# JGCRI/xanthos

Measured on AMD Instinct MI355X. Metric: cell-months/sec (pm_abcd_mrtm, 67,420 cells), higher is better.
Workload: dtype f64

## Files before the change

### xanthos_amd/csrc/xh_flow_rsum.cpp

```cpp
#include <algorithm>
#include <cstdio>
#include <numeric>
#include <string>
#include <thread>

#include "xh_flow_plan.h"

using xh_flow::Tree;
using xh_flow::tree_analyse;

namespace {

constexpr int LANES = 64;
constexpr int G_MAX = 16;
constexpr int W_MAX = 9;
constexpr int SK_P = 4;
constexpr unsigned SK_ZERO = 2u * LANES * 16u;
constexpr int H_MAX = 88;

struct RPart {
    std::vector<int> queue, piece, roots, psize, pimp, pdepth;
    std::vector<int> e_prod, e_cons, e_kind;
    std::vector<int> unit_of_piece, unit_cells, unit_imp, unit_out, unit_depth;
    std::vector<char> unit_cheap, unit_special, special, mayfire;
    int nunit = 0, nedge = 0, maxdepth = 0, n_cheap = 0;
    int n_special = -1;
};

void rsum_partition(const Tree &t, const FlowPlanOptions &opt, int cap, RPart &P, std::vector<int> &fold_leaf) {
    const int n = t.n;
    const std::vector<int> &ds = t.ds, &child = t.child, &child_ptr = t.child_ptr;
    P = RPart();
    std::vector<int> &queue = P.queue;
    queue.reserve(n);
// ... 279 lines not shown
    for (int pass = 0; pass < 4 && need > 0 && opt.foldable; ++pass) {
        std::vector<int> gain(npiece, 0);
        for (int c : queue) {
            const int q = P.piece[c];
            if (q < 0 || special[c] || fold_leaf[c] >= 0 || P.pimp[q] != 0) continue;
            for (int k = child_ptr[c]; k < child_ptr[c + 1]; ++k)
                if (opt.foldable[child[k]] && t.nchild[child[k]] == 0 && P.piece[child[k]] == q) {
                    gain[q]++;
                    break;
                }
        }
        std::vector<int> order;
        for (int p = 0; p < npiece; ++p)
            if (gain[p] > 0) order.push_back(p);
        std::stable_sort(order.begin(), order.end(), [&](int x, int y) { return gain[x] > gain[y]; });
        const int want = (need + 1) * LANES + LANES / 2;
        std::vector<char> chosen(npiece, 0);
        int got = 0;
        for (int p : order) {
            if (got >= want) break;
            chosen[p] = 1;
            got += gain[p];
        }
        if (got == 0) break;
        fold_pieces([&](int p) { return chosen[p] != 0; });
        mark_folds();
        need = pack(false);
    }
    if (need > 0) pack(true);
}

}

int flow_rsum_planner_version() { return 8; }

int flow_tables_build_rsum(int n, const int64_t *indptr, const int32_t *indices, const int8_t *sign, const int *comp,
                           int ncomp, const FlowPlanOptions &opt, std::vector<char> &handled, FlowTables &out,
                           std::string &err) {
    out = FlowTables();
    out.rsum = true;
    handled.assign(n, 0);
    if (n == 0) return 0;
    Tree t;
    tree_analyse(n, indptr, indices, sign, comp, ncomp, t);
    const std::vector<int> &ds = t.ds;

    RPart P;
    std::vector<int> fold_leaf;
    {
        static const int caps[] = {LANES, 56, 48, 44, 40, 36, 32, 28, 24};
        constexpr int NCAP = (int)(sizeof(caps) / sizeof(caps[0]));
        std::vector<RPart> cand(opt.piece_cap > 0 ? 1 : NCAP);
        std::vector<std::vector<int>> cand_fold(cand.size());
        if (cand.size() == 1 || n < 4096) {
            for (size_t k = 0; k < cand.size(); ++k)
                rsum_partition(t, opt, opt.piece_cap > 0 ? std::min(opt.piece_cap, LANES) : caps[k], cand[k], cand_fold[k]);
        } else {
            std::vector<std::thread> pool;
            for (size_t k = 0; k < cand.size(); ++k) pool.emplace_back([&, k] { rsum_partition(t, opt, caps[k], cand[k], cand_fold[k]); });
            for (auto &th : pool) th.join();
        }
        bool have = false;
        long best_score = 0;
        for (size_t k = 0; k < cand.size(); ++k) {
            RPart &Q = cand[k];
            int indep = 0;
            for (int u = 0; u < Q.nunit; ++u) indep += (Q.unit_imp[u] == 0 && Q.unit_out[u] == 0) ? 1 : 0;
// ... 185 lines not shown
    out.n_edges = nedge;
    out.depth = P.maxdepth + 1;
    out.n_cells = (int)std::count(handled.begin(), handled.end(), (char)1);
    out.max_imports = *std::max_element(P.unit_imp.begin(), P.unit_imp.end());
    out.max_exports = *std::max_element(unit_exp.begin(), unit_exp.end());
    out.edge_prod_cell = P.e_prod;
    out.edge_cons_cell = P.e_cons;
    out.unit_depth = P.unit_depth;
    out.piece_of_cell = piece;
    out.unit_of_cell.assign(n, -1);
    for (int c = 0; c < n; ++c)
        if (piece[c] >= 0) out.unit_of_cell[c] = unit_of_piece[piece[c]];
    out.height_of_cell = hgt;
    out.ds = ds;

    if (opt.debug) {
        std::vector<int> hs(4, 0), hl(14, 0), hi(6, 0);
        int indep = 0;
        for (int u = 0; u < nunit; ++u) {
            hs[out.unit_p[u] & 3]++;
            hl[std::min(out.unit_lmax[u] / 16, 13)]++;
            hi[P.unit_imp[u] == 0 ? 0 : P.unit_imp[u] <= 2 ? 1 : P.unit_imp[u] <= 4 ? 2 : P.unit_imp[u] <= 8 ? 3 : 4]++;
            indep += (P.unit_imp[u] == 0 && unit_exp[u] == 0) ? 1 : 0;
        }
        fprintf(stderr, "flow plan (reassociated): %d units (%d without streams, %d kept cheap), %d pieces, %d streams, depth %d, %lld of %lld lanes used\n",
                nunit, indep, P.n_cheap, (int)roots.size(), nedge, P.maxdepth + 1, (long long)out.n_cells, (long long)ts);
        {
            int nfu = 0, nfi = 0;
            for (int u = 0; u < nunit; ++u) {
                nfu += (out.unit_p[u] & 4) ? 1 : 0;
                nfi += ((out.unit_p[u] & 4) && (P.unit_imp[u] > 0 || unit_exp[u] > 0)) ? 1 : 0;
            }
            fprintf(stderr, "  folded leaves: %d, in %d units (of them with streams: %d)\n", out.n_folded, nfu, nfi);
        }
        {
            int nsu = 0;
            for (int u = 0; u < nunit; ++u) nsu += (out.unit_p[u] & 16) ? 1 : 0;
            int nx = 0;
            for (int c = 0; c < n; ++c) nx += (P.n_special >= 0 && P.mayfire[c]) ? 1 : 0;
            int quiet = 0;
            for (int u = 0; u < nunit && P.n_special >= 0; ++u) {
                bool any = (out.unit_p[u] & 16) != 0;
                for (int k = 0; k < LANES && !any; ++k) any = (out.lane_flags[(int64_t)u * LANES + k] & 1) != 0;
                quiet += any ? 0 : 1;
            }
            for (int u = 0; u < nunit && P.n_special >= 0; ++u)
                if (out.unit_p[u] & 16)
                    fprintf(stderr, "  pair unit %d: %d cells, %d imports, %d outlets, depth %d, lmax %d\n", u, P.unit_cells[u], P.unit_imp[u], unit_exp[u],
                            P.unit_depth[u], out.unit_lmax[u]);
            fprintf(stderr, "  single-sum plan: %s, %d cells may fire, %d of them in pair form in %d units; %d single units hold no cell that may fire\n",
                    P.n_special >= 0 ? "yes" : "no", nx, std::max(P.n_special, 0), nsu, quiet);
        }
        fprintf(stderr, "  units by reads (none, A, R, A+R): %d %d %d %d\n  units by lmax/16 (0..13+):", hs[0], hs[1], hs[2], hs[3]);
        for (int k = 0; k < 14; ++k) fprintf(stderr, " %d", hl[k]);
        fprintf(stderr, "\n  units by imports (0, <=2, <=4, <=8, more): %d %d %d %d %d\n  longest stream jump: %d levels\n", hi[0], hi[1],
                hi[2], hi[3], hi[4], out.skew_span);
    }
    return 0;
}

std::string flow_tables_check_rsum(int n, const int64_t *indptr, const int32_t *indices, const int8_t *sign,
                                   const std::vector<char> &handled, const FlowTables &t) {
    if (!t.rsum) return "not a reassociated plan";
    if (t.n_units == 0) {
        for (int c = 0; c < n; ++c)
            if (handled[c]) return "handled cell without units";
// ... 167 lines not shown
```

### xanthos_amd/csrc/xh_mrtm.hip

```cpp
#include <algorithm>
#include <chrono>
#include <climits>
#include <cmath>
#include <atomic>
#include <numeric>
#include <thread>

#include "xh_common.h"
#include <sys/stat.h>
#include <unistd.h>

#include "xh_mrtm_flow.h"
#include "xh_mrtm_plan.h"

namespace {

constexpr int W_MAX = 9;
constexpr int W_BASE = 3;
constexpr int UNIT_MAX_CELLS = 3072;
constexpr int BIN_CELLS = 256;
constexpr int N_CLASS = XH_ROUTE_N_CLASS;

struct UnitClass {
    int nt, kc;
// ... 677 lines not shown
    info[2] = plan->n_units;
    info[3] = plan->fb.n;
    info[4] = plan->largest_unit;
    info[5] = plan->total_slots;
    info[6] = plan->fb_all.single_ds ? 1 : 0;
    const FlowPlan *exact = plan->form[XH_FORM_EXACT].fp, *rsum = last_reassoc(plan);
    int64_t fi[5];
    flow_plan_info(rsum ? rsum : exact, fi);
    info[7] = fi[0];
    info[8] = fi[1];
    info[9] = fi[2];
    info[10] = fi[3];
    info[11] = fi[4];
    info[12] = rsum ? rsum->skew_lmax : ((exact && exact->skew_ok) ? exact->skew_lmax : -1);
    info[13] = plan->last.kernel;
    info[14] = plan->reroutes;
    info[15] = plan->validated;
    return XH_OK;
}

extern "C" int xh_route_plan_stats(xh_route_plan *plan, int64_t max_words, uint64_t *h_words, int64_t *n_words) {
    if (!plan || !n_words) return XH_ERR_ARG;
    std::vector<unsigned long long> st;
    const FlowPlan *rsum = last_reassoc(plan);
    int rc = flow_stats_fetch(plan->ctx, const_cast<FlowPlan *>(rsum ? rsum : plan->form[XH_FORM_EXACT].fp), st);
    if (rc) return rc;
    *n_words = (int64_t)st.size();
    if (h_words)
        for (int64_t i = 0; i < (int64_t)st.size() && i < max_words; ++i) h_words[i] = st[i];
    return XH_OK;
}

constexpr double CAPABLE_THRESHOLD = 1.0 - 1.0 / 1048576.0;

void xh_route_confirm(const xh_route_record &r) { r.plan->fault_streak = 0; }

extern "C" int xh_route_plan_prepare(xh_ctx *ctx, xh_route_plan *plan, const double *h_flow_dist, const double *h_velocity,
                                     double dt) {
    if (!ctx || !plan) return XH_ERR_ARG;
    XH_REQUIRE(ctx, plan->ctx == ctx, "xh_route_plan_prepare: plan belongs to another context");
    XH_REQUIRE(ctx, h_flow_dist && h_velocity && dt > 0.0, "xh_route_plan_prepare: bad argument");
    XH_HIP(ctx, hipSetDevice(ctx->device));
    if (reassoc_wanted(0)) {
        static const bool fold_on = xh_env_on("XH_FLOW_FOLD", true), single_on = xh_env_on("XH_RSUM_SINGLE", true);
        if ((!fold_on && !single_on) || !plan->form[XH_FORM_EXACT].fp || plan->h_indptr.empty()) return XH_OK;
        const size_t n = (size_t)plan->ncell;
        std::vector<unsigned char> foldable(n, 0), capable(n, 0);
        size_t nfold = 0;
        uint64_t key = XH_FNV_BASIS;
        for (size_t c = 0; c < n; ++c) {
            const double tauinv = h_velocity[c] / h_flow_dist[c];
            const bool leaf = plan->h_indptr[c + 1] - plan->h_indptr[c] == 1;
            capable[c] = (tauinv * dt <= CAPABLE_THRESHOLD) ? 0 : 1;
            foldable[c] = (leaf && tauinv >= 0.0 && tauinv * dt <= CAPABLE_THRESHOLD) ? 1 : 0;
            nfold += foldable[c];
            const unsigned char sets = (unsigned char)(capable[c] | (foldable[c] << 1));
            key = xh_fnv1a(key, &sets, 1);
        }
        key = xh_fnv1a(key, &dt, sizeof(dt));
        if (key == 0) key = 1;
        if (plan->fold_tried && key == plan->prep_key) return XH_OK;
        RouteForm &prepared = plan->form[XH_FORM_PREPARED];
        if (prepared.fp) {
            XH_HIP(ctx, hipStreamSynchronize(ctx->stream));
            if (plan->last.fp == prepared.fp) {
                plan->last.form = XH_FORM_EXACT;
                plan->last.fp = nullptr;
            }
            flow_plan_destroy(prepared.fp);
            prepared.fp = nullptr;
            prepared.first_checked = false;
        }
        plan->fold_tried = true;
        plan->prep_key = key;
        plan->fold_disabled = false;
        const bool fold = fold_on && nfold > 0;
        if (!fold && !single_on) return XH_OK;
        const int rcu = rsum_partition(ctx, plan, fold ? foldable.data() : nullptr, single_on ? capable.data() : nullptr,
                                       &prepared.fp);
        if (rcu || !prepared.fp) return rcu;
        prepared.suffix = prepared.fp->n_special >= 0 ? "_rs" : "_rf";
        plan->fold_dt = dt;
        return XH_OK;
    }
    return XH_OK;
}

// ... 254 lines not shown
```

### xanthos_amd/csrc/xh_mrtm_flow.hip

```cpp

#include <algorithm>
#include <cmath>
#include <cstdlib>
#include <numeric>

#include "xh_flow_plan.h"
#include "xh_mrtm_flow.h"

namespace {

constexpr int W_MAX = 9;
constexpr int LANES = 64;
constexpr int NPAIR = 2 * LANES + 1;
constexpr int RING = 4;
constexpr int PF = 8;
constexpr unsigned FAULT_DATA_WAIT = 1, FAULT_RING_WAIT = 2;
constexpr unsigned FAULT_TEST = 99;
constexpr unsigned long long SPIN_LIMIT_TICKS = 500000000ull;

struct FlowArgs {
    const int *cell_of_slot;
    const unsigned *ent;
    const int *export_edge;
    const int *ghost_edge;
// ... 217 lines not shown
int put(xh_ctx *ctx, FlowBuf &b, const std::vector<T> &v) {
    XH_HIP(ctx, hipMalloc(&b.p, v.empty() ? 16 : v.size() * sizeof(T)));
    if (!v.empty()) XH_HIP(ctx, hipMemcpy(b.p, v.data(), v.size() * sizeof(T), hipMemcpyHostToDevice));
    return XH_OK;
}

}

void flow_plan_destroy(FlowPlan *fp) {
    if (!fp) return;
    FlowBuf *bufs[] = {&fp->d_cell_of_slot, &fp->d_ent,      &fp->d_export_edge, &fp->d_ghost_edge,
                       &fp->d_edge_cons_unit, &fp->d_unit_terms, &fp->d_lag,        &fp->d_ghost_lag,
                       &fp->d_ent2,         &fp->d_eprev,       &fp->d_unit_order,  &fp->d_unit_p,     &fp->d_unit_lmax,   &fp->d_unit_glmax,
                       &fp->d_lane_flags,   &fp->d_fold_cell};
    for (FlowBuf *b : bufs)
        if (b->p) (void)hipFree(b->p);
    if (fp->d_x) (void)hipFree(fp->d_x);
    if (fp->d_skew_args) (void)hipFree(fp->d_skew_args);
    if (fp->d_stats) (void)hipFree(fp->d_stats);
    delete fp;
}

void flow_plan_info(const FlowPlan *fp, int64_t info[5]) {
    info[0] = fp ? fp->n_units : 0;
    info[1] = fp ? fp->n_edges : 0;
    info[2] = fp ? fp->depth : 0;
    info[3] = fp ? fp->n_cells : 0;
    info[4] = fp ? fp->max_imports : 0;
}

FlowPlanOptions flow_plan_options(const xh_ctx *ctx) {
    FlowPlanOptions o;
    o.simds = 4 * (ctx->prop.multiProcessorCount > 0 ? ctx->prop.multiProcessorCount : 0);
    if (const char *e = getenv("XH_FLOW_PIECE_CAP")) o.piece_cap = std::min(std::max(atoi(e), 1), LANES);
    o.debug = xh_flow_debug();
    return o;
}

int flow_tables_host(FlowPlanOptions opt, int n, const int64_t *indptr, const int32_t *indices, const int8_t *sign,
                     const std::vector<int> &comp, int ncomp, std::vector<char> &handled, FlowTables &t, std::string &err) {
    handled.assign(n, 0);
    t = FlowTables();
    if (n == 0) return 0;
    opt.capable = nullptr;
    if (flow_tables_build(n, indptr, indices, sign, comp.data(), ncomp, opt, handled, t, err) != 0) return -1;
    if (t.n_units == 0) return 0;
    if (xh_flow_check()) {
        const std::string bad = flow_tables_check(n, indptr, indices, sign, handled, t);
        if (!bad.empty()) {
            err = "flow plan check: " + bad;
            return -1;
        }
    }
    return 0;
}

int flow_tables_cached(const char *name, int n, const int64_t *indptr, const int32_t *indices, const int8_t *sign, bool rsum,
                       bool folds, bool singles, FlowTables &t, std::vector<char> &handled,
                       const std::function<int(FlowTables &, std::vector<char> &)> &build) {
    const std::string path = name ? xh_cache_path(name, false) : std::string();
    if (!path.empty() && flow_tables_load(path.c_str(), t) && t.rsum == rsum && t.n_units > 0 &&
        (int64_t)t.cell_of_slot.size() == (int64_t)t.n_units * LANES && (folds || t.n_folded == 0) && (singles || t.n_special < 0)) {
        handled.assign((size_t)n, 0);
        bool ok = true;
        for (const std::vector<int> *cells : {&t.cell_of_slot, &t.fold_of_slot})
            for (int c : *cells) {
// ... 160 lines not shown
```

### xanthos_amd/csrc/xh_mrtm_rsum.hip

```cpp
#include <algorithm>
#include "xh_mrtm_wave_unit.h"

namespace {

__global__ void __launch_bounds__(LANES) __attribute__((amdgpu_waves_per_eu(2, 2))) k_mrtm_rsum(const WaveArgs *ap_) {
    WaveArgsK *ap = (WaveArgsK *)ap_;
    __shared__ __attribute__((aligned(16))) v2d lds[RING * NSLOT];
    __shared__ uint2 xtab[LANES];
    __shared__ unsigned qstage_sh[4 * LANES];
    __shared__ double fend_sh[2 * LANES];
    __shared__ int unit_sh, prio_sh;
    const int unit = wave_claim(ap, &unit_sh, &prio_sh);
    const int prio = prio_sh;
    if (unit < 0) return;
    if (A(months_ready)) {
        if (prio == 3) __builtin_amdgcn_s_setprio(3);
        else if (prio == 1) __builtin_amdgcn_s_setprio(1);
        else __builtin_amdgcn_s_setprio(2);
    } else if (prio == 3) {
        __builtin_amdgcn_s_setprio(3);
    }
    const int p = A(unit_p)[unit];
    const bool has_ghost = A(ghost_edge)[(int64_t)unit * LANES + threadIdx.x] >= 0;
    const bool g = __any(has_ghost), g2 = __any(has_ghost && threadIdx.x >= 8);
    const int nxo = __popcll(__ballot(A(export_edge)[(int64_t)unit * LANES + threadIdx.x] >= 0));
    const bool x = nxo > 0;
    char *l = reinterpret_cast<char *>(lds);
    __attribute__((address_space(3))) unsigned *qst = (__attribute__((address_space(3))) unsigned *)qstage_sh;
    __attribute__((address_space(3))) double *fnd = (__attribute__((address_space(3))) double *)fend_sh;
    fend_sh[threadIdx.x] = 0.0;
    fend_sh[LANES + threadIdx.x] = 0.0;
    if ((p & ~31) != 0x400) {
        if (threadIdx.x == 0) __hip_atomic_store(A(fault), FAULT_PLACE_WAIT, __ATOMIC_RELAXED, __HIP_MEMORY_SCOPE_AGENT);
        return;
    }
    bool bad = false;
#define XH_BY_OUTLETS(...)                                                                 \
    do {                                                                                   \
        if (nxo > 8) wave_unit<__VA_ARGS__, -1>(ap, l, xtab, qst, fnd, unit);              \
        else if (x) wave_unit<__VA_ARGS__, 1>(ap, l, xtab, qst, fnd, unit);                \
        else wave_unit<__VA_ARGS__, 0>(ap, l, xtab, qst, fnd, unit);                       \
    } while (0)
    if (p & 16) {
        if (!(p & 8) || (p & 4)) bad = true;
        else if (g2) XH_BY_OUTLETS(1, 0, 2, true, true, false, 2);
        else if (g) XH_BY_OUTLETS(1, 0, 1, true, true, false, 2);
        else XH_BY_OUTLETS(1, 0, 0, true, true, false, 2);
#undef XH_BY_OUTLETS
    } else if (p & 8) {
        if (p & 4) {
            if (g || !A(fold_cell)) bad = true;
            else wave_unit<1, 0, 0, true, true, true, 1>(ap, l, xtab, qst, fnd, unit);
        } else if (g2) wave_unit<1, 0, 2, true, true, false, 1>(ap, l, xtab, qst, fnd, unit);
        else if (g) wave_unit<1, 0, 1, true, true, false, 1>(ap, l, xtab, qst, fnd, unit);
        else if ((p & 2) || x) wave_unit<1, 0, 0, true, true, false, 1>(ap, l, xtab, qst, fnd, unit);
        else if (p & 1) wave_unit<1, 0, 0, false, true, false, 1>(ap, l, xtab, qst, fnd, unit);
        else wave_unit<0, 0, 0, false, true, false, 1>(ap, l, xtab, qst, fnd, unit);
    } else if (p & 4) {
        if (g || !A(fold_cell)) bad = true;
        else wave_unit<1, 0, 0, true, true, true>(ap, l, xtab, qst, fnd, unit);
    } else if (g2) wave_unit<1, 0, 2, true, true>(ap, l, xtab, qst, fnd, unit);
    else if (g) wave_unit<1, 0, 1, true, true>(ap, l, xtab, qst, fnd, unit);
    else if ((p & 2) || x) wave_unit<1, 0, 0, true, true>(ap, l, xtab, qst, fnd, unit);
    else if (p & 1) wave_unit<1, 0, 0, false, true>(ap, l, xtab, qst, fnd, unit);
    else wave_unit<0, 0, 0, false, true>(ap, l, xtab, qst, fnd, unit);
    if (bad && threadIdx.x == 0)
        __hip_atomic_store(A(fault), FAULT_PLACE_WAIT, __ATOMIC_RELAXED, __HIP_MEMORY_SCOPE_AGENT);
}
#undef A

}

const void *wave_rsum_kernel() { return reinterpret_cast<const void *>(&k_mrtm_rsum); }
```

### xanthos_amd/csrc/xh_mrtm_wave_unit.h

```cpp
#pragma once
#include <algorithm>
#include <climits>
#include <cstdlib>
#include <type_traits>

#include "xh_mrtm_flow.h"

namespace {


constexpr int LANES = 64;
constexpr int SK_P = 4;
#ifndef XH_WAVE_MIDZONE
#define XH_WAVE_MIDZONE 1
#endif
#ifndef XH_WAVE_BMOV
#define XH_WAVE_BMOV 1
#endif
constexpr int NSLOT = 2 * LANES + 1;
constexpr int RING = 8;
constexpr int GROUP = 16;
constexpr int SK_R = 2;
#ifndef XH_WAVE_CH
#define XH_WAVE_CH 256
// ... 116 lines not shown
template <int PRE, int POST, int NG, bool CHAIN, bool RSUM = false, bool FOLD = false, int SGL = 0, int NXR = -1>
__device__ __forceinline__ void wave_unit(WaveArgsK *ap, char *lds_generic, uint2 *xtab,
                                          __attribute__((address_space(3))) unsigned *qstage,
                                          __attribute__((address_space(3))) double *fend, const int unit) {
    constexpr bool HAS_G = NG > 0;
    constexpr bool V8 = SGL == 1;
    typedef Val<V8> V;
    typedef typename V::T val_t;
    typedef typename V::lds_c lds_cv;
    typedef typename V::lds_m lds_mv;
    constexpr unsigned VB = V::B;
    constexpr unsigned SLOTB = NSLOT * VB;
    lds_char *lds0 = (lds_char *)lds_generic;
    const int lane = threadIdx.x;
    const int64_t slot = (int64_t)unit * LANES + lane;

    const int gc = A(cell_of_slot)[slot];
    const bool valid = gc >= 0;
    const int gc_safe = valid ? gc : 0;
    const unsigned row_off = (unsigned)gc_safe * A(q_row_stride);
    const double tauinv = valid ? A(velocity)[gc] / A(flow_dist)[gc] : 0.0;
    const double acoef = 1.0 - tauinv * A(dt);
    const double area = valid ? A(area)[gc] : 0.0;
    const double S0v = (valid && A(S0)) ? A(S0)[gc] : 0.0;
    auto ent_off = [](unsigned o) { return V8 ? o >> 1 : o; };
    static_assert(!RSUM || (PRE <= 1 && POST == 0), "reassociated form: one inflow entry");
    static_assert(!FOLD || (RSUM && NG == 0), "folded leaves: reassociated form, units without imports");
    static_assert(SGL == 0 || RSUM, "single-sum plans: reassociated form");
    const int gcL = FOLD ? A(fold_cell)[slot] : -1;
    const bool validL = FOLD && valid && gcL >= 0;
    const unsigned row_offL = (unsigned)(validL ? gcL : 0) * A(q_row_stride);
    const double tauL = validL ? A(velocity)[gcL] / A(flow_dist)[gcL] : 0.0;
    const double acoefL = 1.0 - tauL * A(dt);
    const double areaL = validL ? A(area)[gcL] : 0.0;
    const double S0L = (validL && A(S0)) ? A(S0)[gcL] : 0.0;
    double SL = 0.0, favgL = 0.0, erlL = 0.0, erlL_n = 0.0, snapSL = 0.0, snapAL = 0.0, FL = 0.0;
    constexpr double FOLD_EPS = 1e-6;
    unsigned gfold = (validL && !(tauL * A(dt) <= 1.0 - 1.0 / 1048576.0 && tauL >= 0.0 && S0L >= 0.0)) ? 1u : 0u;
    constexpr double SGL_EPS = 1e-6;
    constexpr double SGL_XEPS = 1e-10;
    unsigned gsgl = 0;
    bool xlane = false;
    double fmin_seen = 0.0;
    if (SGL != 0) {
        const unsigned lf = A(lane_flags)[slot];
        xlane = valid && (lf & 2u) != 0;
        gsgl = (valid && (!(tauinv >= 0.0) || (!(tauinv * A(dt) <= 1.0 - 1.0 / 1048576.0) && !(lf & 1u)) || S0v < 0.0)) ? 1u : 0u;
    }
    constexpr int PRE_N = PRE > 0 ? PRE : 1, POST_N = POST > 0 ? POST : 1;
    lds_cchar *epre[PRE_N], *epost[POST_N];
#pragma unroll
    for (int w = 0; w < PRE; ++w) epre[w] = lds0 + ent_off(A(ent2)[(int64_t)w * A(total_slots) + slot]);
#pragma unroll
    for (int w = 0; w < POST; ++w) epost[w] = lds0 + ent_off(A(ent2)[(int64_t)(SK_P + w) * A(total_slots) + slot]);
    lds_cchar *eprv = lds0 + (CHAIN ? ent_off(A(eprev)[slot]) : 0u);
    lds_mv *own = (lds_mv *)lds0 + lane;
    const int xedge = A(export_edge)[slot];
    const int gedge = A(ghost_edge)[slot];
    const bool has_x = xedge >= 0, has_g = gedge >= 0;
    const unsigned long long xmask = __ballot(has_x), gmask = __ballot(has_g);
    const int nx_out = __popcll(xmask), ng = __popcll(gmask);
    static_assert(NXR >= -1 && NXR <= 1, "outlet rounds known at compile time: none or one");
    const bool any_x = NXR < 0 ? xmask != 0 : NXR > 0, any_g = HAS_G;
    const int lmax = A(unit_lmax)[unit], glmax = A(unit_glmax)[unit];
    const int lag_g = has_g ? A(ghost_lag)[slot] : 0;
    const unsigned *ready_p = A(ready) + (has_g ? gedge : 0);
    const unsigned *done_p = A(done) + (has_x ? A(edge_cons_unit)[xedge] : 0);
    const unsigned maskb = A(ring_mask_b);
    const unsigned oob = ~maskb;
    const __amdgpu_buffer_rsrc_t xr = __builtin_amdgcn_make_buffer_rsrc(A(xbuf), 0, (int)A(xbytes), 0x00020000);
    const int total = A(total), nit = A(nit);
// ... 99 lines not shown
    constexpr int OB = 4;
    double ob_s[OB], ob_a[OB];
    double ob_sL[FOLD ? OB : 1], ob_aL[FOLD ? OB : 1];
#pragma unroll
    for (int j = 0; j < OB; ++j) ob_s[j] = ob_a[j] = 0.0;
#pragma unroll
    for (int j = 0; j < (FOLD ? OB : 1); ++j) ob_sL[j] = ob_aL[j] = 0.0;
    bool alive = true;
    unsigned mready = A(ready_at_launch);
    auto wait_months = [&](unsigned need) {
        const unsigned *p = A(months_ready);
        if (!p) return true;
        const unsigned long long t0 = __builtin_amdgcn_s_memrealtime();
        for (;;) {
            unsigned v = 0;
            if (lane == 0) v = __hip_atomic_fetch_add(const_cast<unsigned *>(p), 0u, __ATOMIC_RELAXED, __HIP_MEMORY_SCOPE_AGENT);
            v = (unsigned)__builtin_amdgcn_readfirstlane((int)v);
            if (v >= need) {
                mready = v;
                return true;
            }
            if (ld_relaxed(A(fault)) != 0) return false;
            if (__builtin_amdgcn_s_memrealtime() - t0 > SPIN_LIMIT_TICKS) {
                __hip_atomic_store(A(fault), FAULT_DATA_WAIT, __ATOMIC_RELAXED, __HIP_MEMORY_SCOPE_AGENT);
                return false;
            }
            __builtin_amdgcn_s_sleep(16);
        }
    };
    unsigned long long cyc_wait_data = 0, cyc_wait_ring = 0, zone_groups = 0;
    const unsigned long long cyc_begin = __builtin_amdgcn_s_memtime();
    const unsigned long long rt_begin = __builtin_amdgcn_s_memrealtime();

    unsigned seen_ready = 0, seen_done = 0, pend_ready = 0, pend_done = 0;
    auto load_async = [&](const unsigned *q) {
        unsigned v;
        asm volatile("global_load_dword %0, %1, off sc1" : "=v"(v) : "v"(q) : "memory");
        return v;
    };
    auto check = [&](int n) {
        const unsigned long long w0 = __builtin_amdgcn_s_memtime();
        asm volatile("s_waitcnt vmcnt(8)" : "+v"(pend_ready), "+v"(pend_done) : : "memory");
        asm volatile("s_waitcnt vmcnt(0)" ::: "memory");
        if (SGL == 2) gsgl |= (xlane && fmin_seen < -SGL_XEPS) ? 4u : 0u;
        if ((FOLD && __any(gfold != 0)) || (SGL != 0 && __any(gsgl != 0))) {
            __hip_atomic_store(A(fault), FAULT_GUARD, __ATOMIC_RELAXED, __HIP_MEMORY_SCOPE_AGENT);
            alive = false;
        }
        const bool fenced = A(fenced) == 1;
        if (any_x) {
            const int pub = min(max(n - RING - lmax, 0), total);
            if (fenced) __builtin_amdgcn_fence(__ATOMIC_RELEASE, "agent");
            if (has_x) __hip_atomic_store(A(ready) + xedge, (unsigned)pub, __ATOMIC_RELAXED, __HIP_MEMORY_SCOPE_AGENT);
            const int need = n + CH - lmax - A(rs);
            seen_done = max(seen_done, pend_done);
            if (need > 0 && alive)
                alive = wave_wait_ge(has_x, done_p, (unsigned)min(need, total), seen_done, A(fault), FAULT_RING_WAIT);
        }
        const unsigned long long w1 = __builtin_amdgcn_s_memtime();
        if (any_g && alive) {
            if (lane == 0)
                __hip_atomic_store(A(done) + unit, (unsigned)min(max(n - glmax, 0), total), __ATOMIC_RELAXED,
                                   __HIP_MEMORY_SCOPE_AGENT);
            const int need = min(total, n + CH + GROUP - lag_g);
            seen_ready = max(seen_ready, pend_ready);
            alive = wave_wait_ge(has_g && need > 0, ready_p, (unsigned)max(need, 0), seen_ready, A(fault), FAULT_DATA_WAIT);
            if (fenced) __builtin_amdgcn_fence(__ATOMIC_ACQUIRE, "agent");
            asm volatile("" ::: "memory");
        }
        if (any_x) pend_done = load_async(done_p);
        if (any_g) pend_ready = load_async(ready_p);
        cyc_wait_ring += w1 - w0;
        cyc_wait_data += __builtin_amdgcn_s_memtime() - w1;
    };

    auto finalize = [&](int it) {
        const FinRec f = fc;
        fc = ld_fin(it + 1 <= nit ? it + 1 : nit + 1);
        if (it + 1 < nit) {
            const double qn = runoff_take();
            erl_n = ((valid ? qn : 0.0) * area) * 1000.0 / f.secs_next1;
            if (RSUM) erl_n *= dt;
            if (SGL != 0) gsgl |= (erl_n < -SGL_EPS) ? 2u : 0u;
            if (FOLD) {
                const unsigned lo = qstage[2 * LANES + lane], hi = qstage[3 * LANES + lane];
                const double qnL = __hiloint2double((int)hi, (int)lo);
                erlL_n = (((validL ? qnL : 0.0) * areaL) * 1000.0 / f.secs_next1) * dt;
            }
        }
        if (it >= 1) {
            const int m = f.m_prev_w & (FIN_WRITE - 1);
            const bool write_prev = (f.m_prev_w & FIN_WRITE) != 0;
#pragma unroll
            for (int j = 0; j < OB - 1; ++j) {
                ob_s[j] = ob_s[j + 1];
                ob_a[j] = ob_a[j + 1];
            }
            ob_s[OB - 1] = snapS;
            ob_a[OB - 1] = snapA / (double)f.nt_prev;
            if (FOLD) {
#pragma unroll
                for (int j = 0; j < OB - 1; ++j) {
                    ob_sL[j] = ob_sL[j + 1];
                    ob_aL[j] = ob_aL[j + 1];
// ... 83 lines not shown
                import_drop(r, gbuf[b][r]);
                gbuf[b][r] = import_load(r);
            }
        }
        if (any_x) {
            xb[0] = *xsrc[0];
            if (x2) xb[1] = *xsrc[1];
        }
    };
    auto store_pair = [&](const val_t v, unsigned voff, unsigned soff) {
        v2d p;
        if constexpr (SGL == 1) p = v2d{v, v};
        else p = v;
        __builtin_amdgcn_raw_buffer_store_b128(__builtin_bit_cast(v4u, p), xr, voff, soff, AUX_SC1);
    };
    auto block_store = [&](int m0) {
        if (any_x) {
            const unsigned xpos = ((unsigned)(m0 - RING - lmax) * 16u) & maskb;
            store_pair(xb[0], xbyte[0], xpos);
            if (x2) store_pair(xb[1], xbyte[1], xpos);
        }
    };

    check(0);
#pragma unroll
    for (int r = 0; r < SK_R; ++r) gbuf[0][r] = r < NG ? import_load(r) : v4u{0u, 0u, 0u, 0u};
#pragma unroll
    for (int r = 0; r < SK_R; ++r) gbuf[1][r] = r < NG ? import_load(r) : v4u{0u, 0u, 0u, 0u};

    const int N = (total + lmax + 1 + GROUP - 1) & ~(GROUP - 1);
    int itz = 0, gz = 0;
    int itf = 0, nf = (lmax + 1 + GROUP - 1) & ~(GROUP - 1);
    int ntz = nit > 0 ? p_rec[0].nt : 0;

    auto substep = [&](auto zone_c, auto mid_c, const int n, const int j, const int edge, const int rel) {
        constexpr bool MID = decltype(mid_c)::value;
        if (decltype(zone_c)::value && ((j & 1) == 0 || (!MID && odd_ok))) {
            const bool c = rel == j;
#if XH_WAVE_BMOV
            {
                const unsigned long long cm = __ballot(c);
                unsigned long long sv;
                asm volatile("s_and_saveexec_b64 %[sv], %[cm]\n\tv_mov_b64 %[ss], %[s]\n\tv_mov_b64 %[sa], %[fa]\n\t"
                             "v_mov_b64 %[fa], 0\n\tv_mov_b64 %[e], %[en]\n\ts_mov_b64 exec, %[sv]"
                             : [ss] "+v"(snapS), [sa] "+v"(snapA), [fa] "+v"(favg), [e] "+v"(erl), [sv] "=&s"(sv)
                             : [s] "v"(S), [en] "v"(erl_n), [cm] "s"(cm)
                             : "scc");
            }
#else
            snapS = c ? S : snapS;
            snapA = c ? favg : snapA;

            favg = c ? 0.0 : favg;
            erl = c ? erl_n : erl;
#endif
            if (FOLD) {
                snapSL = c ? SL : snapSL;
                snapAL = c ? favgL : snapAL;
                favgL = c ? 0.0 : favgL;
                erlL = c ? erlL_n : erlL;
            }
            if (!MID) {
                if (edge == 1) S = c ? S0v : S;
                if (FOLD && edge == 1) SL = c ? S0L : SL;
                if (edge == 2) {
                    if (c) fend[lane] = F;
                    if (FOLD && c) fend[LANES + lane] = FL;
                }
            }
        }
        __builtin_amdgcn_sched_barrier(0);
        val_t(&ac)[PRE_N] = va[j & 1], (&bc)[POST_N] = vb[j & 1], (&an)[PRE_N] = va[(j & 1) ^ 1], (&bn)[POST_N] = vb[(j & 1) ^ 1];
        const val_t rc = vr[j & 1];
        const unsigned so = (unsigned)((j + RING - 1) & (RING - 1)) * SLOTB;
        if (CHAIN) vr[(j & 1) ^ 1] = *(lds_cv *)(eprv + so);
#pragma unroll
        for (int w = 0; w < PRE; ++w) an[w] = *(lds_cv *)(epre[w] + so);
#pragma unroll
        for (int w = 0; w < POST; ++w) bn[w] = *(lds_cv *)(epost[w] + so);
        __builtin_amdgcn_sched_barrier(0);
        __builtin_amdgcn_s_waitcnt(0xC07F | ((PRE + POST + (CHAIN ? 1 : 0) + 1) << 8));
        __builtin_amdgcn_sched_barrier(0);
        if ((j & (RING - 1)) == 0) block_io(j / RING);
        if ((j & (RING - 1)) == 1) block_store(n + j - 1);
        const double F0 = S * tauinv;
        if constexpr (RSUM) {
            double base = __builtin_fma(S, acoef, erl);
            if (FOLD) {
                FL = SL * tauL;
                SL = __builtin_fma(SL, acoefL, erlL);
                favgL += FL;
                base = __builtin_fma(FL, dt, base);
            }
            if constexpr (SGL == 1) {
                const double S1 = PRE ? __builtin_fma(ac[0], dt, base) : base;
                const double m = __builtin_fmin(S1, 0.0);
                const double f2 = __builtin_fma(m, dtinv, F0);
                own[(j & (RING - 1)) * NSLOT] = CHAIN ? rc + f2 : f2;
                S = S1 - m;
                F = f2;
                favg += f2;
            } else {
            const double S1 = PRE ? __builtin_fma(ac[0].x, dt, base) : base;
            const double S2 = PRE ? __builtin_fma(ac[0].y, dt, base) : base;
            const bool sx = S1 < 0.0;
            const double f2 = __builtin_fma(__builtin_fmin(S1, 0.0), dtinv, F0);
            own[(j & (RING - 1)) * NSLOT] = CHAIN ? v2d{rc.x + F0, rc.y + f2} : v2d{F0, f2};
            double Sn = S2;
            asm volatile("" : "+v"(Sn));
            S = sx ? 0.0 : Sn;
            F = f2;
            favg += f2;
            if (SGL == 2) fmin_seen = __builtin_fmin(fmin_seen, f2);
            }
        } else {
            double s1 = 0.0, s2 = 0.0;
#pragma unroll
            for (int w = 0; w < PRE; ++w) {
                s1 += ac[w].x;
                s2 += ac[w].y;
            }
            s1 -= F0;
#pragma unroll
            for (int w = 0; w < POST; ++w) s1 += bc[w].x;
            const double dsdt = s1 + erl;
// ... 5 lines not shown
            for (int w = 0; w < POST; ++w) s2 += bc[w].y;
            const double dsdt2 = s2 + erl;
            double Sn = S + dsdt2 * dt;
            asm volatile("" : "+v"(Sn));
            S = sx ? 0.0 : Sn;
            F = f2;
            favg += f2;
        }
    };

#ifdef XH_WAVE_PROFILE
    unsigned long long prof_zone = 0, prof_fin = 0, prof_t = __builtin_amdgcn_s_memtime();
#define PROF_MARK(acc)                                                  \
    {                                                                   \
        const unsigned long long now_ = __builtin_amdgcn_s_memtime();   \
        acc += now_ - prof_t;                                           \
        prof_t = now_;                                                  \
    }
    unsigned long long prof_plain = 0;
#else
#define PROF_MARK(acc)
#endif
    auto housekeeping = [&](int n) {
        if (n > 0 && (n & (CH - 1)) == 0) check(n);
        if (alive && n == nf) {
            const int g_next = finalize(itf);
            ++itf;
            nf = itf <= nit ? ((g_next + lmax + 1 + GROUP - 1) & ~(GROUP - 1)) : INT_MAX;
        }
        PROF_MARK(prof_fin)
    };
    int n = 0;
    while (n < N && alive) {
        if (itz <= nit && n + GROUP > gz && n <= gz + lmax) {
            const int edge = itz == 0 ? 1 : (itz == nit ? 2 : 0);
            auto zone_run = [&](auto mid_c) {
                do {
                    housekeeping(n);
                    if (!alive) break;
                    ++zone_groups;
                    const int rel = nx - n;
#pragma unroll
                    for (int j = 0; j < GROUP; ++j) substep(std::true_type(), mid_c, n, j, edge, rel);
                    n += GROUP;
                    PROF_MARK(prof_zone)
                } while (n <= gz + lmax && n < N);
            };
#if XH_WAVE_MIDZONE
            if (edge == 0 && !odd_ok) zone_run(std::true_type());
            else zone_run(std::false_type());
#else
            zone_run(std::false_type());
#endif
            if (alive) {
                nx = itz < nit ? nx + ntz : INT_MAX;
                ++itz;
                gz = p_rec[itz <= nit ? itz : nit].g;
                if (itz > nit) gz = INT_MAX;
                ntz = p_rec[itz <= nit ? itz : nit].nt;
            }
        } else {
            const int n_end = itz <= nit ? min(N, gz & ~(GROUP - 1)) : N;
            do {
                housekeeping(n);
                if (!alive) break;
#pragma unroll
                for (int j = 0; j < GROUP; ++j) substep(std::false_type(), std::false_type(), n, j, 0, 0);
                n += GROUP;
                PROF_MARK(prof_plain)
            } while (n < n_end);
        }
    }
    if (alive) {
        while (itf <= nit) finalize(itf++);
        if (SGL == 2) gsgl |= (xlane && fmin_seen < -SGL_XEPS) ? 4u : 0u;
        if ((FOLD && __any(gfold != 0)) || (SGL != 0 && __any(gsgl != 0))) {
            __hip_atomic_store(A(fault), FAULT_GUARD, __ATOMIC_RELAXED, __HIP_MEMORY_SCOPE_AGENT);
            alive = false;
        }
    }
    if (alive) {
        if (any_x) {
            const unsigned xpos = ((unsigned)(N - RING - lmax) * 16u) & maskb;
            store_pair(*xsrc[0], xbyte[0], xpos);
            if (x2) store_pair(*xsrc[1], xbyte[1], xpos);
            asm volatile("s_waitcnt vmcnt(0)" ::: "memory");
            if (A(fenced) == 1) __builtin_amdgcn_fence(__ATOMIC_RELEASE, "agent");
            if (has_x) __hip_atomic_store(A(ready) + xedge, (unsigned)total, __ATOMIC_RELAXED, __HIP_MEMORY_SCOPE_AGENT);
        }
        if (any_g && lane == 0)
            __hip_atomic_store(A(done) + unit, (unsigned)total, __ATOMIC_RELAXED, __HIP_MEMORY_SCOPE_AGENT);
        if (valid) {
            if (A(S_end)) A(S_end)[gc] = snapS;
            if (A(F_end)) A(F_end)[gc] = fend[lane];
        }
// ... 131 lines not shown
```

Baseline: 3.184 billion.

## Derive folded-leaf average flow algebraically and poll counters on demand

The folded-leaf update no longer computes and accumulates the leaf flow every substep. The per-month average is recovered from the storage balance (nt*inflow minus storage change), and the leaf contribution is applied as a single fma on the leaf storage. The flow is only recomputed in the zone before the final month, which needs an extra group on the last zone. Folding now also requires tauinv*dt above 1/65536, to keep the algebraic average well conditioned. The asynchronous prefetch of ring and data counters is replaced by conditional relaxed loads issued only when the cached values are not already sufficient. Folded-unit dispatch is also routed through the outlet-specialised macro, and debug and env knobs are added.

```diff
diff --git a/xanthos_amd/csrc/xh_flow_rsum.cpp b/xanthos_amd/csrc/xh_flow_rsum.cpp
--- a/xanthos_amd/csrc/xh_flow_rsum.cpp
+++ b/xanthos_amd/csrc/xh_flow_rsum.cpp
@@ -1,5 +1,6 @@
 #include <algorithm>
 #include <cstdio>
+#include <cstdlib>
 #include <numeric>
 #include <string>
 #include <thread>
@@ -345,7 +346,7 @@
 
 }
 
-int flow_rsum_planner_version() { return 8; }
+int flow_rsum_planner_version() { return 9; }
 
 int flow_tables_build_rsum(int n, const int64_t *indptr, const int32_t *indices, const int8_t *sign, const int *comp,
                            int ncomp, const FlowPlanOptions &opt, std::vector<char> &handled, FlowTables &out,
@@ -597,6 +598,17 @@
                 nfi += ((out.unit_p[u] & 4) && (P.unit_imp[u] > 0 || unit_exp[u] > 0)) ? 1 : 0;
             }
             fprintf(stderr, "  folded leaves: %d, in %d units (of them with streams: %d)\n", out.n_folded, nfu, nfi);
+            int ho[2][3] = {{0, 0, 0}, {0, 0, 0}};
+            for (int u = 0; u < nunit; ++u) ho[(out.unit_p[u] & 4) ? 1 : 0][unit_exp[u] == 0 ? 0 : unit_exp[u] <= 8 ? 1 : 2]++;
+            fprintf(stderr, "  units by outlets (0, <=8, more): %d %d %d; of them with folded leaves: %d %d %d\n", ho[0][0] + ho[1][0],
+                    ho[0][1] + ho[1][1], ho[0][2] + ho[1][2], ho[1][0], ho[1][1], ho[1][2]);
+            const char *lvl = getenv("XH_FLOW_DEBUG");
+            if (lvl && atoi(lvl) >= 2) {
+                fprintf(stderr, "  folded cells:");
+                for (int c : out.fold_of_slot)
+                    if (c >= 0) fprintf(stderr, " %d", c);
+                fprintf(stderr, "\n");
+            }
         }
         {
             int nsu = 0;
diff --git a/xanthos_amd/csrc/xh_mrtm.hip b/xanthos_amd/csrc/xh_mrtm.hip
--- a/xanthos_amd/csrc/xh_mrtm.hip
+++ b/xanthos_amd/csrc/xh_mrtm.hip
@@ -733,6 +733,7 @@
 }
 
 constexpr double CAPABLE_THRESHOLD = 1.0 - 1.0 / 1048576.0;
+constexpr double FOLDABLE_MIN = 1.0 / 65536.0;
 
 void xh_route_confirm(const xh_route_record &r) { r.plan->fault_streak = 0; }
 
@@ -753,7 +754,7 @@
             const double tauinv = h_velocity[c] / h_flow_dist[c];
             const bool leaf = plan->h_indptr[c + 1] - plan->h_indptr[c] == 1;
             capable[c] = (tauinv * dt <= CAPABLE_THRESHOLD) ? 0 : 1;
-            foldable[c] = (leaf && tauinv >= 0.0 && tauinv * dt <= CAPABLE_THRESHOLD) ? 1 : 0;
+            foldable[c] = (leaf && tauinv >= 0.0 && tauinv * dt <= CAPABLE_THRESHOLD && tauinv * dt >= FOLDABLE_MIN) ? 1 : 0;
             nfold += foldable[c];
             const unsigned char sets = (unsigned char)(capable[c] | (foldable[c] << 1));
             key = xh_fnv1a(key, &sets, 1);
diff --git a/xanthos_amd/csrc/xh_mrtm_flow.hip b/xanthos_amd/csrc/xh_mrtm_flow.hip
--- a/xanthos_amd/csrc/xh_mrtm_flow.hip
+++ b/xanthos_amd/csrc/xh_mrtm_flow.hip
@@ -273,6 +273,7 @@
 FlowPlanOptions flow_plan_options(const xh_ctx *ctx) {
     FlowPlanOptions o;
     o.simds = 4 * (ctx->prop.multiProcessorCount > 0 ? ctx->prop.multiProcessorCount : 0);
+    if (const char *e = getenv("XH_FLOW_SIMDS")) o.simds = std::max(atoi(e), 0);
     if (const char *e = getenv("XH_FLOW_PIECE_CAP")) o.piece_cap = std::min(std::max(atoi(e), 1), LANES);
     o.debug = xh_flow_debug();
     return o;
diff --git a/xanthos_amd/csrc/xh_mrtm_rsum.hip b/xanthos_amd/csrc/xh_mrtm_rsum.hip
--- a/xanthos_amd/csrc/xh_mrtm_rsum.hip
+++ b/xanthos_amd/csrc/xh_mrtm_rsum.hip
@@ -46,19 +46,18 @@
         else if (g2) XH_BY_OUTLETS(1, 0, 2, true, true, false, 2);
         else if (g) XH_BY_OUTLETS(1, 0, 1, true, true, false, 2);
         else XH_BY_OUTLETS(1, 0, 0, true, true, false, 2);
-#undef XH_BY_OUTLETS
     } else if (p & 8) {
         if (p & 4) {
             if (g || !A(fold_cell)) bad = true;
-            else wave_unit<1, 0, 0, true, true, true, 1>(ap, l, xtab, qst, fnd, unit);
-        } else if (g2) wave_unit<1, 0, 2, true, true, false, 1>(ap, l, xtab, qst, fnd, unit);
-        else if (g) wave_unit<1, 0, 1, true, true, false, 1>(ap, l, xtab, qst, fnd, unit);
-        else if ((p & 2) || x) wave_unit<1, 0, 0, true, true, false, 1>(ap, l, xtab, qst, fnd, unit);
+            else XH_BY_OUTLETS(1, 0, 0, true, true, true, 1);
+        } else if (g2) XH_BY_OUTLETS(1, 0, 2, true, true, false, 1);
+        else if (g) XH_BY_OUTLETS(1, 0, 1, true, true, false, 1);
+        else if ((p & 2) || x) XH_BY_OUTLETS(1, 0, 0, true, true, false, 1);
         else if (p & 1) wave_unit<1, 0, 0, false, true, false, 1>(ap, l, xtab, qst, fnd, unit);
         else wave_unit<0, 0, 0, false, true, false, 1>(ap, l, xtab, qst, fnd, unit);
     } else if (p & 4) {
         if (g || !A(fold_cell)) bad = true;
-        else wave_unit<1, 0, 0, true, true, true>(ap, l, xtab, qst, fnd, unit);
+        else XH_BY_OUTLETS(1, 0, 0, true, true, true, 0);
     } else if (g2) wave_unit<1, 0, 2, true, true>(ap, l, xtab, qst, fnd, unit);
     else if (g) wave_unit<1, 0, 1, true, true>(ap, l, xtab, qst, fnd, unit);
     else if ((p & 2) || x) wave_unit<1, 0, 0, true, true>(ap, l, xtab, qst, fnd, unit);
@@ -67,6 +66,7 @@
     if (bad && threadIdx.x == 0)
         __hip_atomic_store(A(fault), FAULT_PLACE_WAIT, __ATOMIC_RELAXED, __HIP_MEMORY_SCOPE_AGENT);
 }
+#undef XH_BY_OUTLETS
 #undef A
 
 }
diff --git a/xanthos_amd/csrc/xh_mrtm_wave_unit.h b/xanthos_amd/csrc/xh_mrtm_wave_unit.h
--- a/xanthos_amd/csrc/xh_mrtm_wave_unit.h
+++ b/xanthos_amd/csrc/xh_mrtm_wave_unit.h
@@ -172,11 +172,13 @@
     const unsigned row_offL = (unsigned)(validL ? gcL : 0) * A(q_row_stride);
     const double tauL = validL ? A(velocity)[gcL] / A(flow_dist)[gcL] : 0.0;
     const double acoefL = 1.0 - tauL * A(dt);
+    const double kL = tauL * A(dt);
     const double areaL = validL ? A(area)[gcL] : 0.0;
     const double S0L = (validL && A(S0)) ? A(S0)[gcL] : 0.0;
-    double SL = 0.0, favgL = 0.0, erlL = 0.0, erlL_n = 0.0, snapSL = 0.0, snapAL = 0.0, FL = 0.0;
+    double SL = 0.0, erlL = 0.0, erlL_n = 0.0, snapSL = 0.0, snapAL = 0.0, FL = 0.0;
     constexpr double FOLD_EPS = 1e-6;
-    unsigned gfold = (validL && !(tauL * A(dt) <= 1.0 - 1.0 / 1048576.0 && tauL >= 0.0 && S0L >= 0.0)) ? 1u : 0u;
+    constexpr double FOLD_MIN = 1.0 / 65536.0;
+    unsigned gfold = (validL && !(kL <= 1.0 - 1.0 / 1048576.0 && kL >= FOLD_MIN && tauL >= 0.0 && S0L >= 0.0)) ? 1u : 0u;
     constexpr double SGL_EPS = 1e-6;
     constexpr double SGL_XEPS = 1e-10;
     unsigned gsgl = 0;
@@ -342,15 +344,14 @@
     const unsigned long long cyc_begin = __builtin_amdgcn_s_memtime();
     const unsigned long long rt_begin = __builtin_amdgcn_s_memrealtime();
 
-    unsigned seen_ready = 0, seen_done = 0, pend_ready = 0, pend_done = 0;
-    auto load_async = [&](const unsigned *q) {
-        unsigned v;
-        asm volatile("global_load_dword %0, %1, off sc1" : "=v"(v) : "v"(q) : "memory");
-        return v;
-    };
+    unsigned seen_ready = 0, seen_done = 0;
     auto check = [&](int n) {
         const unsigned long long w0 = __builtin_amdgcn_s_memtime();
-        asm volatile("s_waitcnt vmcnt(8)" : "+v"(pend_ready), "+v"(pend_done) : : "memory");
+        const int need_x = min(n + CH - lmax - A(rs), total), need_g = min(total, n + CH + GROUP - lag_g);
+        unsigned now_done = 0u, now_ready = 0u;
+        if (any_x && !__all(!has_x || need_x <= 0 || seen_done >= (unsigned)need_x)) now_done = ld_relaxed(done_p);
+        if (any_g && !__all(!has_g || need_g <= 0 || seen_ready >= (unsigned)need_g)) now_ready = ld_relaxed(ready_p);
+        asm volatile("s_waitcnt vmcnt(8)" ::: "memory");
         asm volatile("s_waitcnt vmcnt(0)" ::: "memory");
         if (SGL == 2) gsgl |= (xlane && fmin_seen < -SGL_XEPS) ? 4u : 0u;
         if ((FOLD && __any(gfold != 0)) || (SGL != 0 && __any(gsgl != 0))) {
@@ -363,7 +364,7 @@
             if (fenced) __builtin_amdgcn_fence(__ATOMIC_RELEASE, "agent");
             if (has_x) __hip_atomic_store(A(ready) + xedge, (unsigned)pub, __ATOMIC_RELAXED, __HIP_MEMORY_SCOPE_AGENT);
             const int need = n + CH - lmax - A(rs);
-            seen_done = max(seen_done, pend_done);
+            seen_done = max(seen_done, now_done);
             if (need > 0 && alive)
                 alive = wave_wait_ge(has_x, done_p, (unsigned)min(need, total), seen_done, A(fault), FAULT_RING_WAIT);
         }
@@ -373,13 +374,11 @@
                 __hip_atomic_store(A(done) + unit, (unsigned)min(max(n - glmax, 0), total), __ATOMIC_RELAXED,
                                    __HIP_MEMORY_SCOPE_AGENT);
             const int need = min(total, n + CH + GROUP - lag_g);
-            seen_ready = max(seen_ready, pend_ready);
+            seen_ready = max(seen_ready, now_ready);
             alive = wave_wait_ge(has_g && need > 0, ready_p, (unsigned)max(need, 0), seen_ready, A(fault), FAULT_DATA_WAIT);
             if (fenced) __builtin_amdgcn_fence(__ATOMIC_ACQUIRE, "agent");
             asm volatile("" ::: "memory");
         }
-        if (any_x) pend_done = load_async(done_p);
-        if (any_g) pend_ready = load_async(ready_p);
         cyc_wait_ring += w1 - w0;
         cyc_wait_data += __builtin_amdgcn_s_memtime() - w1;
     };
@@ -529,6 +528,7 @@
     int itz = 0, gz = 0;
     int itf = 0, nf = (lmax + 1 + GROUP - 1) & ~(GROUP - 1);
     int ntz = nit > 0 ? p_rec[0].nt : 0;
+    double nt_zone = 0.0;
 
     auto substep = [&](auto zone_c, auto mid_c, const int n, const int j, const int edge, const int rel) {
         constexpr bool MID = decltype(mid_c)::value;
@@ -552,14 +552,16 @@
             erl = c ? erl_n : erl;
 #endif
             if (FOLD) {
+                snapAL = c ? (nt_zone * erlL - (SL - snapSL)) * dtinv : snapAL;
                 snapSL = c ? SL : snapSL;
-                snapAL = c ? favgL : snapAL;
-                favgL = c ? 0.0 : favgL;
                 erlL = c ? erlL_n : erlL;
             }
             if (!MID) {
                 if (edge == 1) S = c ? S0v : S;
-                if (FOLD && edge == 1) SL = c ? S0L : SL;
+                if (FOLD && edge == 1) {
+                    SL = c ? S0L : SL;
+                    snapSL = c ? S0L : snapSL;
+                }
                 if (edge == 2) {
                     if (c) fend[lane] = F;
                     if (FOLD && c) fend[LANES + lane] = FL;
@@ -584,10 +586,9 @@
         if constexpr (RSUM) {
             double base = __builtin_fma(S, acoef, erl);
             if (FOLD) {
-                FL = SL * tauL;
+                if (decltype(zone_c)::value && !MID) FL = SL * tauL;
+                base = __builtin_fma(SL, kL, base);
                 SL = __builtin_fma(SL, acoefL, erlL);
-                favgL += FL;
-                base = __builtin_fma(FL, dt, base);
             }
             if constexpr (SGL == 1) {
                 const double S1 = PRE ? __builtin_fma(ac[0], dt, base) : base;
@@ -659,7 +660,8 @@
     };
     int n = 0;
     while (n < N && alive) {
-        if (itz <= nit && n + GROUP > gz && n <= gz + lmax) {
+        const int gz_lo = (FOLD && itz == nit) ? gz - GROUP : gz;
+        if (itz <= nit && n + GROUP > gz_lo && n <= gz + lmax) {
             const int edge = itz == 0 ? 1 : (itz == nit ? 2 : 0);
             auto zone_run = [&](auto mid_c) {
                 do {
@@ -681,13 +683,14 @@
 #endif
             if (alive) {
                 nx = itz < nit ? nx + ntz : INT_MAX;
+                if (FOLD) nt_zone = (double)ntz;
                 ++itz;
                 gz = p_rec[itz <= nit ? itz : nit].g;
                 if (itz > nit) gz = INT_MAX;
                 ntz = p_rec[itz <= nit ? itz : nit].nt;
             }
         } else {
-            const int n_end = itz <= nit ? min(N, gz & ~(GROUP - 1)) : N;
+            const int n_end = itz <= nit ? min(N, gz_lo & ~(GROUP - 1)) : N;
             do {
                 housekeeping(n);
                 if (!alive) break;
```

Result: no change. 3.201 billion, median of 6 (+0.5%).
